# Xjh-UCAS/TAM-TR

Hardware: AMD Instinct MI355X
Metric: images/sec fwd+bwd @640x640 bs=16/GPU (higher is better)
Workload: dtype bf16

## Files before the change

### tam-tr_amd/csrc/bn.hip

```cpp
#include "common.h"

namespace {

constexpr int BN_THREADS = 256;
constexpr int BN_EPT = 16;
constexpr int BN_SLICE = BN_THREADS * BN_EPT;

template <typename T>
__device__ __forceinline__ void ld_slice(const T* __restrict__ p, int n, bool vec, float (&v)[BN_EPT], int (&cnt)) {
  const int base = threadIdx.x * BN_EPT;
  cnt = max(0, min(BN_EPT, n - base));
  if (vec && cnt == BN_EPT) {
#pragma unroll
    for (int q = 0; q < BN_EPT / 4; ++q) {
      float o[4];
      Elt<T>::ld4(p + base + 4 * q, o);
      v[4 * q] = o[0]; v[4 * q + 1] = o[1]; v[4 * q + 2] = o[2]; v[4 * q + 3] = o[3];
    }
  } else {
#pragma unroll
    for (int i = 0; i < BN_EPT; ++i) v[i] = i < cnt ? Elt<T>::ld(p + base + i) : 0.f;
  }
}

// ... 133 lines not shown
    }
  } else {
    for (int i = 0; i < cnt; ++i) Elt<T>::st(y + off + base + i, act_fwd(fmaf(Elt<T>::ld(x + off + base + i) - mean, a, be), act));
  }
}

template <typename T>
__global__ __launch_bounds__(BN_THREADS) void bn_bwd_reduce_kernel(const T* __restrict__ gy, const T* __restrict__ x,
                                                                    const float* __restrict__ mean_rstd, const float* __restrict__ gamma,
                                                                    const float* __restrict__ beta, float* __restrict__ part, int C,
                                                                    int HW, int vec, int act) {
  __shared__ float s_red[BN_THREADS / WAVE];
  const int s = blockIdx.x, c = blockIdx.y, b = blockIdx.z, S = gridDim.x * gridDim.z;
  const int n = min(BN_SLICE, HW - s * BN_SLICE);
  const size_t off = ((size_t)b * C + c) * HW + (size_t)s * BN_SLICE;
  const float mean = mean_rstd[2 * c], rstd = mean_rstd[2 * c + 1], g = gamma[c], be = beta[c];
  float xv[BN_EPT], gv[BN_EPT];
  int cnt;
  ld_slice<T>(x + off, n, vec, xv, cnt);
  ld_slice<T>(gy + off, n, vec, gv, cnt);
  float s1 = 0.f, s2 = 0.f;
#pragma unroll
  for (int i = 0; i < BN_EPT; ++i) {
    if (i < cnt) {
      const float xh = (xv[i] - mean) * rstd;
      const float dz = gv[i] * act_bwd(fmaf(xh, g, be), act);
      s1 += dz;
      s2 = fmaf(dz, xh, s2);
    }
  }
  s1 = block_sum(s1, s_red);
  s2 = block_sum(s2, s_red);
  if (threadIdx.x == 0) {
    float* o = part + ((size_t)c * S + (size_t)b * gridDim.x + s) * 2;
    o[0] = s1; o[1] = s2;
  }
}

template <typename T>
__global__ __launch_bounds__(BN_THREADS) void bn_bwd_apply_kernel(const T* __restrict__ gy, const T* __restrict__ x,
                                                                   const float* __restrict__ mean_rstd, const float* __restrict__ gamma,
                                                                   const float* __restrict__ beta, const float* __restrict__ part,
                                                                   T* __restrict__ gx, float* __restrict__ ggamma, float* __restrict__ gbeta,
                                                                   int C, int HW, int vec, int act, float inv_count) {
  __shared__ float s_red[BN_THREADS / WAVE];
  const int s = blockIdx.x, c = blockIdx.y, b = blockIdx.z, S = gridDim.x * gridDim.z;
  float p1 = 0.f, p2 = 0.f;
  for (int i = threadIdx.x; i < S; i += BN_THREADS) { p1 += part[((size_t)c * S + i) * 2]; p2 += part[((size_t)c * S + i) * 2 + 1]; }
  const float sum_dz = block_sum(p1, s_red), sum_dzx = block_sum(p2, s_red);
  if (s == 0 && b == 0 && threadIdx.x == 0) { ggamma[c] = sum_dzx; gbeta[c] = sum_dz; }
  const int n = min(BN_SLICE, HW - s * BN_SLICE);
  const size_t off = ((size_t)b * C + c) * HW + (size_t)s * BN_SLICE;
  const float mean = mean_rstd[2 * c], rstd = mean_rstd[2 * c + 1], g = gamma[c], be = beta[c];
  const float k1 = sum_dz * inv_count, k2 = sum_dzx * inv_count, gr = g * rstd;
  const int base = threadIdx.x * BN_EPT;
  const int cnt = max(0, min(BN_EPT, n - base));
  if (vec && cnt == BN_EPT) {
#pragma unroll
    for (int q = 0; q < BN_EPT / 4; ++q) {
      float xv[4], gv[4], o[4];
      Elt<T>::ld4(x + off + base + 4 * q, xv);
      Elt<T>::ld4(gy + off + base + 4 * q, gv);
#pragma unroll
      for (int i = 0; i < 4; ++i) {
        const float xh = (xv[i] - mean) * rstd;
        const float dz = gv[i] * act_bwd(fmaf(xh, g, be), act);
        o[i] = gr * (dz - k1 - xh * k2);
      }
      Elt<T>::st4(gx + off + base + 4 * q, o);
    }
  } else {
    for (int i = 0; i < cnt; ++i) {
      const float xh = (Elt<T>::ld(x + off + base + i) - mean) * rstd;
      const float dz = Elt<T>::ld(gy + off + base + i) * act_bwd(fmaf(xh, g, be), act);
      Elt<T>::st(gx + off + base + i, gr * (dz - k1 - xh * k2));
    }
  }
}

template <typename T, int V>
struct Vec;
template <>
struct Vec<float, 4> {
  static __device__ __forceinline__ void ld(const float* p, float (&o)[4]) { Elt<float>::ld4(p, o); }
  static __device__ __forceinline__ void st(float* p, const float (&v)[4]) { Elt<float>::st4(p, v); }
};
template <>
struct Vec<bf16_t, 4> {
  static __device__ __forceinline__ void ld(const bf16_t* p, float (&o)[4]) { Elt<bf16_t>::ld4(p, o); }
  static __device__ __forceinline__ void st(bf16_t* p, const float (&v)[4]) { Elt<bf16_t>::st4(p, v); }
};
template <>
struct Vec<bf16_t, 8> {
  static __device__ __forceinline__ void ld(const bf16_t* p, float (&o)[8]) {
    const uint4 t = *reinterpret_cast<const uint4*>(p);
    const uint32_t w[4] = {t.x, t.y, t.z, t.w};
#pragma unroll
    for (int i = 0; i < 4; ++i) { o[2 * i] = __uint_as_float(w[i] << 16); o[2 * i + 1] = __uint_as_float(w[i] & 0xffff0000u); }
  }
  static __device__ __forceinline__ void st(bf16_t* p, const float (&v)[8]) {
    uint32_t w[4];
#pragma unroll
    for (int i = 0; i < 4; ++i) w[i] = (uint32_t)f2bf(v[2 * i]) | ((uint32_t)f2bf(v[2 * i + 1]) << 16);
    *reinterpret_cast<uint4*>(p) = make_uint4(w[0], w[1], w[2], w[3]);
  }
};

constexpr int CL_UNROLL = 4;

template <int W>
__device__ __forceinline__ void fold_row_lanes(const float (&mine)[W], float* s_acc, float* s_col, int cg) {
#pragma unroll
  for (int j = 0; j < W; ++j) s_acc[threadIdx.x * W + j] = mine[j];
  __syncthreads();
  const int rl = BN_THREADS / cg;
  for (int o = threadIdx.x; o < cg * W; o += BN_THREADS) {
    const int g = o / W, j = o % W;
    float a = 0.f;
    for (int q = 0; q < rl; ++q) a += s_acc[(q * cg + g) * W + j];
    s_col[o] = a;
  }
  __syncthreads();
}

struct Seg { unsigned rows; size_t pitch; };
__device__ __forceinline__ size_t seg_addr(size_t e, int C, int cshift, size_t ld, Seg sg) {
  const size_t row = e >> cshift, col = e & (size_t)(C - 1);
  if (!sg.rows) return row * ld + col;
  const unsigned img = (unsigned)row / sg.rows;
  return (size_t)img * sg.pitch + ((unsigned)row - img * sg.rows) * ld + col;
}

template <typename T, int V>
__global__ __launch_bounds__(BN_THREADS) void bncl_stats_kernel(const T* __restrict__ x, float* __restrict__ part, size_t total, int C,
                                                                 int iters) {
  __shared__ float s_acc[BN_THREADS * 2 * V];
  __shared__ float s_col[2 * 1024];
  const size_t piece = (size_t)BN_THREADS * V, start = (size_t)blockIdx.x * iters * piece, end = min(total, start + iters * piece);
  const int cg = C / V, g = threadIdx.x % cg, S = gridDim.x;
  const T* home = x + start + (size_t)g * V;
  float k[V], acc[2 * V];
  Vec<T, V>::ld(home, k);
#pragma unroll
  for (int j = 0; j < 2 * V; ++j) acc[j] = 0.f;
  const size_t e0 = start + (size_t)threadIdx.x * V;
  for (int it = 0; it < iters; it += CL_UNROLL) {
    float v[CL_UNROLL][V];
#pragma unroll
    for (int u = 0; u < CL_UNROLL; ++u) {
      const size_t e = e0 + (size_t)(it + u) * piece;
      Vec<T, V>::ld(e < end ? x + e : home, v[u]);
    }
#pragma unroll
    for (int u = 0; u < CL_UNROLL; ++u)
#pragma unroll
      for (int j = 0; j < V; ++j) { const float d = v[u][j] - k[j]; acc[j] += d; acc[V + j] = fmaf(d, d, acc[V + j]); }
  }
  fold_row_lanes<2 * V>(acc, s_acc, s_col, cg);
  const float n = (float)((end - start) / C);
  for (int c = threadIdx.x; c < C; c += BN_THREADS) {
    const float s1 = s_col[(c / V) * 2 * V + c % V], s2 = s_col[(c / V) * 2 * V + V + c % V], m = s1 / n;
    float* o = part + ((size_t)c * S + blockIdx.x) * 3;
    o[0] = n; o[1] = Elt<T>::ld(x + start + c) + m; o[2] = s2 - s1 * m;
  }
}

template <typename T, int V>
__global__ __launch_bounds__(BN_THREADS) void bncl_apply_kernel(const T* __restrict__ x, const float* __restrict__ mean_rstd,
                                                                 const float* __restrict__ gamma, const float* __restrict__ beta,
                                                                 const T* __restrict__ res, T* __restrict__ y, size_t total, int C, int iters,
                                                                 int act, Seg ysg = Seg{0, 0}, int cshift = 0) {
  const size_t piece = (size_t)BN_THREADS * V, start = (size_t)blockIdx.x * iters * piece, end = min(total, start + iters * piece);
  const int c0 = (threadIdx.x % (C / V)) * V;
  const size_t home = start + c0;
  float mean[V], a[V], be[V];
#pragma unroll
  for (int j = 0; j < V; ++j) { mean[j] = mean_rstd[2 * (c0 + j)]; a[j] = mean_rstd[2 * (c0 + j) + 1] * gamma[c0 + j]; be[j] = beta[c0 + j]; }
  const size_t e0 = start + (size_t)threadIdx.x * V;
  for (int it = 0; it < iters; it += CL_UNROLL) {
    float v[CL_UNROLL][V];
#pragma unroll
    for (int u = 0; u < CL_UNROLL; ++u) {
      const size_t e = e0 + (size_t)(it + u) * piece;
      Vec<T, V>::ld(x + (e < end ? e : home), v[u]);
    }
#pragma unroll
    for (int u = 0; u < CL_UNROLL; ++u) {
      const size_t e = e0 + (size_t)(it + u) * piece;
#pragma unroll
      for (int j = 0; j < V; ++j) v[u][j] = act_fwd(fmaf(v[u][j] - mean[j], a[j], be[j]), act);
      if (res && e < end) {
        float r[V];
        Vec<T, V>::ld(res + e, r);
#pragma unroll
        for (int j = 0; j < V; ++j) v[u][j] += r[j];
      }
      if (e < end) Vec<T, V>::st(y + (ysg.rows ? seg_addr(e, C, cshift, (size_t)C, ysg) : e), v[u]);
    }
  }
}

template <typename T, int V>
__global__ __launch_bounds__(BN_THREADS) void bncl2_apply_kernel(const T* __restrict__ x1, const T* __restrict__ x2,
                                                                  const float* __restrict__ mr1, const float* __restrict__ mr2,
                                                                  const float* __restrict__ g1, const float* __restrict__ b1,
                                                                  const float* __restrict__ g2, const float* __restrict__ b2,
                                                                  T* __restrict__ y, size_t total, int C, int iters, int act) {
  const size_t piece = (size_t)BN_THREADS * V, start = (size_t)blockIdx.x * iters * piece, end = min(total, start + iters * piece);
  const int c0 = (threadIdx.x % (C / V)) * V;
  const size_t home = start + c0;
  float m1[V], a1[V], m2[V], a2[V], be[V];
#pragma unroll
  for (int j = 0; j < V; ++j) {
    m1[j] = mr1[2 * (c0 + j)]; a1[j] = mr1[2 * (c0 + j) + 1] * g1[c0 + j];
    m2[j] = mr2[2 * (c0 + j)]; a2[j] = mr2[2 * (c0 + j) + 1] * g2[c0 + j];
    be[j] = b1[c0 + j] + b2[c0 + j];
  }
  const size_t e0 = start + (size_t)threadIdx.x * V;
  for (int it = 0; it < iters; it += CL_UNROLL) {
    float v[CL_UNROLL][V], w[CL_UNROLL][V];
#pragma unroll
    for (int u = 0; u < CL_UNROLL; ++u) {
      const size_t e = e0 + (size_t)(it + u) * piece, ee = e < end ? e : home;
      Vec<T, V>::ld(x1 + ee, v[u]);
      Vec<T, V>::ld(x2 + ee, w[u]);
    }
#pragma unroll
    for (int u = 0; u < CL_UNROLL; ++u) {
      const size_t e = e0 + (size_t)(it + u) * piece;
#pragma unroll
      for (int j = 0; j < V; ++j) v[u][j] = act_fwd(fmaf(w[u][j] - m2[j], a2[j], fmaf(v[u][j] - m1[j], a1[j], be[j])), act);
      if (e < end) Vec<T, V>::st(y + e, v[u]);
    }
  }
}

template <typename T, int V>
__global__ __launch_bounds__(BN_THREADS) void bncl2_bwd_reduce_kernel(const T* __restrict__ gy, const T* __restrict__ x1, const T* __restrict__ x2,
                                                                       const float* __restrict__ mr1, const float* __restrict__ mr2,
                                                                       const float* __restrict__ g1, const float* __restrict__ b1,
                                                                       const float* __restrict__ g2, const float* __restrict__ b2,
                                                                       float* __restrict__ part, size_t total, int C, int iters, int act,
                                                                       size_t ldgy, int cshift) {
  __shared__ float s_acc[BN_THREADS * 3 * V];
  __shared__ float s_col[3 * 1024];
  const size_t piece = (size_t)BN_THREADS * V, start = (size_t)blockIdx.x * iters * piece, end = min(total, start + iters * piece);
  const int cg = C / V, c0 = (threadIdx.x % cg) * V, S = gridDim.x;
  const size_t home = start + c0;
  float m1[V], r1[V], m2[V], r2[V], ga1[V], ga2[V], be[V], acc[3 * V];
#pragma unroll
  for (int j = 0; j < V; ++j) {
    m1[j] = mr1[2 * (c0 + j)]; r1[j] = mr1[2 * (c0 + j) + 1]; m2[j] = mr2[2 * (c0 + j)]; r2[j] = mr2[2 * (c0 + j) + 1];
    ga1[j] = g1[c0 + j]; ga2[j] = g2[c0 + j]; be[j] = b1[c0 + j] + b2[c0 + j];
    acc[j] = 0.f; acc[V + j] = 0.f; acc[2 * V + j] = 0.f;
  }
  const size_t e0 = start + (size_t)threadIdx.x * V;
  for (int it = 0; it < iters; it += CL_UNROLL) {
    float xa[CL_UNROLL][V], xb[CL_UNROLL][V], gv[CL_UNROLL][V];
#pragma unroll
    for (int u = 0; u < CL_UNROLL; ++u) {
      const size_t e = e0 + (size_t)(it + u) * piece, ee = e < end ? e : home;
      Vec<T, V>::ld(x1 + ee, xa[u]);
      Vec<T, V>::ld(x2 + ee, xb[u]);
      Vec<T, V>::ld(gy + (ee >> cshift) * ldgy + (ee & (size_t)(C - 1)), gv[u]);
    }
#pragma unroll
    for (int u = 0; u < CL_UNROLL; ++u) {
      const float live = e0 + (size_t)(it + u) * piece < end ? 1.f : 0.f;
#pragma unroll
      for (int j = 0; j < V; ++j) {
        const float h1 = (xa[u][j] - m1[j]) * r1[j], h2 = (xb[u][j] - m2[j]) * r2[j];
        const float dz = live * gv[u][j] * act_bwd(fmaf(h2, ga2[j], fmaf(h1, ga1[j], be[j])), act);
        acc[j] += dz; acc[V + j] = fmaf(dz, h1, acc[V + j]); acc[2 * V + j] = fmaf(dz, h2, acc[2 * V + j]);
      }
    }
  }
  fold_row_lanes<3 * V>(acc, s_acc, s_col, cg);
  for (int c = threadIdx.x; c < C; c += BN_THREADS) {
    float* o = part + ((size_t)c * S + blockIdx.x) * 3;
    o[0] = s_col[(c / V) * 3 * V + c % V]; o[1] = s_col[(c / V) * 3 * V + V + c % V]; o[2] = s_col[(c / V) * 3 * V + 2 * V + c % V];
  }
}

__global__ __launch_bounds__(BN_THREADS) void bncl2_sum_kernel(const float* __restrict__ part, float* __restrict__ sums, float* __restrict__ gg1,
                                                                float* __restrict__ gb1, float* __restrict__ gg2, float* __restrict__ gb2, int S) {
  __shared__ float s_red[BN_THREADS / WAVE];
  const int c = blockIdx.x;
  float a = 0.f, b = 0.f, d = 0.f;
  for (int s = threadIdx.x; s < S; s += BN_THREADS) {
    const float* p = part + ((size_t)c * S + s) * 3;
    a += p[0]; b += p[1]; d += p[2];
  }
  a = block_sum(a, s_red); b = block_sum(b, s_red); d = block_sum(d, s_red);
  if (threadIdx.x == 0) { sums[3 * c] = a; sums[3 * c + 1] = b; sums[3 * c + 2] = d; gb1[c] = a; gb2[c] = a; gg1[c] = b; gg2[c] = d; }
}

template <typename T, int V>
__global__ __launch_bounds__(BN_THREADS) void bncl2_bwd_apply_kernel(const T* __restrict__ gy, const T* __restrict__ x1, const T* __restrict__ x2,
                                                                      const float* __restrict__ mr1, const float* __restrict__ mr2,
                                                                      const float* __restrict__ g1, const float* __restrict__ b1,
                                                                      const float* __restrict__ g2, const float* __restrict__ b2,
                                                                      const float* __restrict__ sums, T* __restrict__ gx1, T* __restrict__ gx2,
                                                                      size_t total, int C, int iters, int act, float inv_count, size_t ldgy,
                                                                      int cshift) {
  const size_t piece = (size_t)BN_THREADS * V, start = (size_t)blockIdx.x * iters * piece, end = min(total, start + iters * piece);
  const int c0 = (threadIdx.x % (C / V)) * V;
  const size_t home = start + c0;
  float m1[V], r1[V], m2[V], r2[V], ga1[V], ga2[V], be[V], k1[V], k2[V], k3[V];
#pragma unroll
  for (int j = 0; j < V; ++j) {
    m1[j] = mr1[2 * (c0 + j)]; r1[j] = mr1[2 * (c0 + j) + 1]; m2[j] = mr2[2 * (c0 + j)]; r2[j] = mr2[2 * (c0 + j) + 1];
    ga1[j] = g1[c0 + j]; ga2[j] = g2[c0 + j]; be[j] = b1[c0 + j] + b2[c0 + j];
    k1[j] = sums[3 * (c0 + j)] * inv_count; k2[j] = sums[3 * (c0 + j) + 1] * inv_count; k3[j] = sums[3 * (c0 + j) + 2] * inv_count;
  }
  const size_t e0 = start + (size_t)threadIdx.x * V;
  for (int it = 0; it < iters; it += CL_UNROLL / 2) {
    float xa[CL_UNROLL / 2][V], xb[CL_UNROLL / 2][V], gv[CL_UNROLL / 2][V];
#pragma unroll
    for (int u = 0; u < CL_UNROLL / 2; ++u) {
      const size_t e = e0 + (size_t)(it + u) * piece, ee = e < end ? e : home;
      Vec<T, V>::ld(x1 + ee, xa[u]);
      Vec<T, V>::ld(x2 + ee, xb[u]);
      Vec<T, V>::ld(gy + (ee >> cshift) * ldgy + (ee & (size_t)(C - 1)), gv[u]);
    }
#pragma unroll
    for (int u = 0; u < CL_UNROLL / 2; ++u) {
      const size_t e = e0 + (size_t)(it + u) * piece;
#pragma unroll
      for (int j = 0; j < V; ++j) {
        const float h1 = (xa[u][j] - m1[j]) * r1[j], h2 = (xb[u][j] - m2[j]) * r2[j];
        const float dz = gv[u][j] * act_bwd(fmaf(h2, ga2[j], fmaf(h1, ga1[j], be[j])), act);
        xa[u][j] = ga1[j] * r1[j] * (dz - k1[j] - h1 * k2[j]);
        xb[u][j] = ga2[j] * r2[j] * (dz - k1[j] - h2 * k3[j]);
      }
      if (e < end) { Vec<T, V>::st(gx1 + e, xa[u]); Vec<T, V>::st(gx2 + e, xb[u]); }
    }
  }
}

template <typename T, int V>
__global__ __launch_bounds__(BN_THREADS) void bncl_bwd_reduce_kernel(const T* __restrict__ gy, const T* __restrict__ x,
                                                                      const float* __restrict__ mean_rstd, const float* __restrict__ gamma,
                                                                      const float* __restrict__ beta, float* __restrict__ part, size_t total,
                                                                      int C, int iters, int act, size_t ldgy, int cshift, Seg gsg = Seg{0, 0}) {
  __shared__ float s_acc[BN_THREADS * 2 * V];
  __shared__ float s_col[2 * 1024];
  const size_t piece = (size_t)BN_THREADS * V, start = (size_t)blockIdx.x * iters * piece, end = min(total, start + iters * piece);
  const int cg = C / V, c0 = (threadIdx.x % cg) * V, S = gridDim.x;
  const size_t home = start + c0;
  float mean[V], rstd[V], gm[V], be[V], acc[2 * V];
#pragma unroll
  for (int j = 0; j < V; ++j) {
    mean[j] = mean_rstd[2 * (c0 + j)]; rstd[j] = mean_rstd[2 * (c0 + j) + 1]; gm[j] = gamma[c0 + j]; be[j] = beta[c0 + j];
    acc[j] = 0.f; acc[V + j] = 0.f;
  }
  const size_t e0 = start + (size_t)threadIdx.x * V;
  for (int it = 0; it < iters; it += CL_UNROLL) {
    float xv[CL_UNROLL][V], gv[CL_UNROLL][V];
#pragma unroll
    for (int u = 0; u < CL_UNROLL; ++u) {
      const size_t e = e0 + (size_t)(it + u) * piece, ee = e < end ? e : home;
      Vec<T, V>::ld(x + ee, xv[u]);
      Vec<T, V>::ld(gy + seg_addr(ee, C, cshift, ldgy, gsg), gv[u]);
    }
#pragma unroll
    for (int u = 0; u < CL_UNROLL; ++u) {
      const float live = e0 + (size_t)(it + u) * piece < end ? 1.f : 0.f;
#pragma unroll
      for (int j = 0; j < V; ++j) {
        const float xh = (xv[u][j] - mean[j]) * rstd[j];
        const float dz = live * gv[u][j] * act_bwd(fmaf(xh, gm[j], be[j]), act);
        acc[j] += dz; acc[V + j] = fmaf(dz, xh, acc[V + j]);
      }
    }
  }
  fold_row_lanes<2 * V>(acc, s_acc, s_col, cg);
  for (int c = threadIdx.x; c < C; c += BN_THREADS) {
    float* o = part + ((size_t)c * S + blockIdx.x) * 2;
    o[0] = s_col[(c / V) * 2 * V + c % V]; o[1] = s_col[(c / V) * 2 * V + V + c % V];
  }
}

__global__ __launch_bounds__(BN_THREADS) void bncl_sum_kernel(const float* __restrict__ part, float* __restrict__ sums, float* __restrict__ ggamma,
                                                               float* __restrict__ gbeta, int S) {
  __shared__ float s_red[BN_THREADS / WAVE];
  const int c = blockIdx.x;
  float a = 0.f, b = 0.f;
  for (int s = threadIdx.x; s < S; s += BN_THREADS) { a += part[((size_t)c * S + s) * 2]; b += part[((size_t)c * S + s) * 2 + 1]; }
  a = block_sum(a, s_red); b = block_sum(b, s_red);
  if (threadIdx.x == 0) { sums[2 * c] = a; sums[2 * c + 1] = b; gbeta[c] = a; ggamma[c] = b; }
}

template <typename T, int V>
__global__ __launch_bounds__(BN_THREADS) void bncl_bwd_apply_kernel(const T* __restrict__ gy, const T* __restrict__ x,
                                                                     const float* __restrict__ mean_rstd, const float* __restrict__ gamma,
                                                                     const float* __restrict__ beta, const float* __restrict__ sums,
                                                                     T* __restrict__ gx, size_t total, int C, int iters, int act,
                                                                     float inv_count, size_t ldgy, int cshift, Seg gsg = Seg{0, 0}) {
  const size_t piece = (size_t)BN_THREADS * V, start = (size_t)blockIdx.x * iters * piece, end = min(total, start + iters * piece);
  const int c0 = (threadIdx.x % (C / V)) * V;
  const size_t home = start + c0;
  float mean[V], rstd[V], gm[V], be[V], k1[V], k2[V];
#pragma unroll
  for (int j = 0; j < V; ++j) {
    mean[j] = mean_rstd[2 * (c0 + j)]; rstd[j] = mean_rstd[2 * (c0 + j) + 1]; gm[j] = gamma[c0 + j]; be[j] = beta[c0 + j];
    k1[j] = sums[2 * (c0 + j)] * inv_count; k2[j] = sums[2 * (c0 + j) + 1] * inv_count;
  }
  const size_t e0 = start + (size_t)threadIdx.x * V;
  for (int it = 0; it < iters; it += CL_UNROLL) {
    float xv[CL_UNROLL][V], gv[CL_UNROLL][V];
#pragma unroll
    for (int u = 0; u < CL_UNROLL; ++u) {
      const size_t e = e0 + (size_t)(it + u) * piece, ee = e < end ? e : home;
      Vec<T, V>::ld(x + ee, xv[u]);
      Vec<T, V>::ld(gy + seg_addr(ee, C, cshift, ldgy, gsg), gv[u]);
    }
#pragma unroll
    for (int u = 0; u < CL_UNROLL; ++u) {
      const size_t e = e0 + (size_t)(it + u) * piece;
#pragma unroll
      for (int j = 0; j < V; ++j) {
        const float xh = (xv[u][j] - mean[j]) * rstd[j];
        const float dz = gv[u][j] * act_bwd(fmaf(xh, gm[j], be[j]), act);
        gv[u][j] = gm[j] * rstd[j] * (dz - k1[j] - xh * k2[j]);
      }
      if (e < end) Vec<T, V>::st(gx + e, gv[u]);
    }
  }
}

}

extern "C" int tamtr_bn_slices(int B, int HW) { return B * ((HW + BN_SLICE - 1) / BN_SLICE); }

static int bn_check(const void* a, const void* b, int B, int C, int HW, int dtype, int act) {
  if (!a || !b || B <= 0 || C <= 0 || HW <= 0) return TAMTR_EINVAL;
  if ((dtype != TAMTR_F32 && dtype != TAMTR_BF16) || (act != 0 && act != 1)) return TAMTR_EINVAL;
  if (B > 65535 || C > 65535) return TAMTR_EUNSUP;
  return TAMTR_OK;
}
static int bn_vec(const void* p, const void* q, int HW, int dtype) {
  const int e = dtype == TAMTR_F32 ? 4 : 2;
  return HW % 4 == 0 && ((uintptr_t)p % (4 * e)) == 0 && (!q || ((uintptr_t)q % (4 * e)) == 0);
}

extern "C" int tamtr_bn_act_fwd(const void* x, const float* gamma, const float* beta, float* running_mean, float* running_var, void* y,
                                float* mean_rstd, float* partials, int B, int C, int HW, float eps, float momentum, int act, int dtype,
                                void* stream) {
  const int rc = bn_check(x, y, B, C, HW, dtype, act);
  if (rc) return rc;
  if (!gamma || !beta || !mean_rstd || !partials) return TAMTR_EINVAL;
  const int sh = (HW + BN_SLICE - 1) / BN_SLICE, vec = bn_vec(x, y, HW, dtype);
  const dim3 grid(sh, C, B);
  hipStream_t s = (hipStream_t)stream;
  if (dtype == TAMTR_F32) hipLaunchKernelGGL(bn_stats_kernel<float>, grid, dim3(BN_THREADS), 0, s, (const float*)x, partials, C, HW, vec);
  else hipLaunchKernelGGL(bn_stats_kernel<bf16_t>, grid, dim3(BN_THREADS), 0, s, (const bf16_t*)x, partials, C, HW, vec);
  if (dtype == TAMTR_F32)
    hipLaunchKernelGGL(bn_apply_kernel<float>, grid, dim3(BN_THREADS), 0, s, (const float*)x, partials, mean_rstd, running_mean, running_var,
                       gamma, beta, (float*)y, C, HW, vec, act, eps, momentum);
  else
    hipLaunchKernelGGL(bn_apply_kernel<bf16_t>, grid, dim3(BN_THREADS), 0, s, (const bf16_t*)x, partials, mean_rstd, running_mean,
                       running_var, gamma, beta, (bf16_t*)y, C, HW, vec, act, eps, momentum);
  return tamtr_launch_status();
}

extern "C" int tamtr_bn_act_bwd(const void* gy, const void* x, const float* gamma, const float* beta, const float* mean_rstd, void* gx,
                                float* ggamma, float* gbeta, float* partials, int B, int C, int HW, int act, int dtype, void* stream) {
  const int rc = bn_check(gy, x, B, C, HW, dtype, act);
  if (rc) return rc;
  if (!gamma || !beta || !mean_rstd || !gx || !ggamma || !gbeta || !partials) return TAMTR_EINVAL;
  const int sh = (HW + BN_SLICE - 1) / BN_SLICE, vec = bn_vec(x, gy, HW, dtype) && bn_vec(gx, nullptr, HW, dtype);
  const dim3 grid(sh, C, B);
  hipStream_t s = (hipStream_t)stream;
  const float inv = 1.f / ((float)B * (float)HW);
  if (dtype == TAMTR_F32) {
    hipLaunchKernelGGL(bn_bwd_reduce_kernel<float>, grid, dim3(BN_THREADS), 0, s, (const float*)gy, (const float*)x, mean_rstd, gamma, beta,
                       partials, C, HW, vec, act);
    hipLaunchKernelGGL(bn_bwd_apply_kernel<float>, grid, dim3(BN_THREADS), 0, s, (const float*)gy, (const float*)x, mean_rstd, gamma, beta,
                       partials, (float*)gx, ggamma, gbeta, C, HW, vec, act, inv);
  } else {
    hipLaunchKernelGGL(bn_bwd_reduce_kernel<bf16_t>, grid, dim3(BN_THREADS), 0, s, (const bf16_t*)gy, (const bf16_t*)x, mean_rstd, gamma,
                       beta, partials, C, HW, vec, act);
    hipLaunchKernelGGL(bn_bwd_apply_kernel<bf16_t>, grid, dim3(BN_THREADS), 0, s, (const bf16_t*)gy, (const bf16_t*)x, mean_rstd, gamma,
                       beta, partials, (bf16_t*)gx, ggamma, gbeta, C, HW, vec, act, inv);
  }
  return tamtr_launch_status();
}

static int bncl_vec(int C, int dtype) { return dtype == TAMTR_BF16 && C % 8 == 0 ? 8 : 4; }
static int bncl_iters(long long N, int C, int dtype) {
  const long long piece = (long long)BN_THREADS * bncl_vec(C, dtype), total = N * C;
  const long long it = (total / piece / 1024 + CL_UNROLL - 1) / CL_UNROLL * CL_UNROLL;
  return (int)(it < 4 ? 4 : it > 64 ? 64 : it);
}
extern "C" int tamtr_bncl_blocks(long long N, int C, int dtype) {
  if (N <= 0 || C <= 0) return 0;
  const long long chunk = (long long)bncl_iters(N, C, dtype) * BN_THREADS * bncl_vec(C, dtype);
  return (int)((N * C + chunk - 1) / chunk);
}

static int bncl_check(const void* a, const void* b, long long N, int C, int dtype, int act) {
  if (!a || !b || N <= 0 || C <= 0) return TAMTR_EINVAL;
  if ((dtype != TAMTR_F32 && dtype != TAMTR_BF16) || (act != 0 && act != 1)) return TAMTR_EINVAL;
  const int cg = C / bncl_vec(C, dtype);
  if (C % 4 || C > 1024 || cg > BN_THREADS || (BN_THREADS % cg) || N > 2000000000LL / C) return TAMTR_EUNSUP;
  if (((uintptr_t)a | (uintptr_t)b) % 16) return TAMTR_EUNSUP;
  return TAMTR_OK;
}

static int bncl_act_fwd_impl(const void* x, const float* gamma, const float* beta, float* running_mean, float* running_var,
                             const void* residual, void* y, float* mean_rstd, float* partials, long long N, int C, float eps,
                             float momentum, int act, int dtype, void* stream, Seg ysg, int cshift) {
  const int rc = bncl_check(x, y, N, C, dtype, act);
  if (rc) return rc;
  if (!gamma || !beta || !mean_rstd || !partials) return TAMTR_EINVAL;
  if (residual && (uintptr_t)residual % 16) return TAMTR_EUNSUP;
  const int S = tamtr_bncl_blocks(N, C, dtype), V = bncl_vec(C, dtype), iters = bncl_iters(N, C, dtype);
  const size_t total = (size_t)N * C;
  hipStream_t s = (hipStream_t)stream;
  if (dtype == TAMTR_F32) hipLaunchKernelGGL((bncl_stats_kernel<float, 4>), dim3(S), dim3(BN_THREADS), 0, s, (const float*)x, partials, total, C, iters);
  else if (V == 8) hipLaunchKernelGGL((bncl_stats_kernel<bf16_t, 8>), dim3(S), dim3(BN_THREADS), 0, s, (const bf16_t*)x, partials, total, C, iters);
  else hipLaunchKernelGGL((bncl_stats_kernel<bf16_t, 4>), dim3(S), dim3(BN_THREADS), 0, s, (const bf16_t*)x, partials, total, C, iters);
  hipLaunchKernelGGL(bn_finalize_kernel, dim3(C), dim3(BN_THREADS), 0, s, partials, mean_rstd, running_mean, running_var, S, eps, momentum);
  if (dtype == TAMTR_F32)
    hipLaunchKernelGGL((bncl_apply_kernel<float, 4>), dim3(S), dim3(BN_THREADS), 0, s, (const float*)x, mean_rstd, gamma, beta, (const float*)residual, (float*)y, total, C, iters, act, ysg, cshift);
  else if (V == 8)
    hipLaunchKernelGGL((bncl_apply_kernel<bf16_t, 8>), dim3(S), dim3(BN_THREADS), 0, s, (const bf16_t*)x, mean_rstd, gamma, beta, (const bf16_t*)residual, (bf16_t*)y, total, C, iters, act, ysg, cshift);
  else
    hipLaunchKernelGGL((bncl_apply_kernel<bf16_t, 4>), dim3(S), dim3(BN_THREADS), 0, s, (const bf16_t*)x, mean_rstd, gamma, beta, (const bf16_t*)residual, (bf16_t*)y, total, C, iters, act, ysg, cshift);
  return tamtr_launch_status();
}

extern "C" int tamtr_bncl_act_fwd(const void* x, const float* gamma, const float* beta, float* running_mean, float* running_var,
                                  const void* residual, void* y, float* mean_rstd, float* partials, long long N, int C, float eps,
                                  float momentum, int act, int dtype, void* stream) {
  return bncl_act_fwd_impl(x, gamma, beta, running_mean, running_var, residual, y, mean_rstd, partials, N, C, eps, momentum, act, dtype, stream,
                           Seg{0, 0}, 0);
}

extern "C" int tamtr_bncl_act_seg_fwd(const void* x, const float* gamma, const float* beta, float* running_mean, float* running_var, void* y,
                                      long long seg_rows, long long seg_pitch, float* mean_rstd, float* partials, long long N, int C, float eps,
                                      float momentum, int act, int dtype, void* stream) {
  if (seg_rows <= 0 || N % seg_rows || seg_pitch < seg_rows * C || seg_pitch % 8 || (C & (C - 1)) || seg_rows > 0x7fffffffLL) return TAMTR_EUNSUP;
  int cshift = 0;
  while ((1 << cshift) < C) ++cshift;
  return bncl_act_fwd_impl(x, gamma, beta, running_mean, running_var, nullptr, y, mean_rstd, partials, N, C, eps, momentum, act, dtype, stream,
                           Seg{(unsigned)seg_rows, (size_t)seg_pitch}, cshift);
}

static int bncl_act_bwd_impl(const void* gy, long long ldgy, const void* x, const float* gamma, const float* beta,
                             const float* mean_rstd, void* gx, float* ggamma, float* gbeta, float* partials, long long N, int C, int act,
                             int dtype, void* stream, Seg gsg) {
  const int rc = bncl_check(gy, x, N, C, dtype, act);
  if (rc) return rc;
  if (ldgy < C || ldgy % bncl_vec(C, dtype) || (C & (C - 1))) return TAMTR_EUNSUP;
  int cshift = 0;
  while ((1 << cshift) < C) ++cshift;
  if (!gamma || !beta || !mean_rstd || !gx || !ggamma || !gbeta || !partials || (uintptr_t)gx % 16) return TAMTR_EINVAL;
  const int S = tamtr_bncl_blocks(N, C, dtype), V = bncl_vec(C, dtype), iters = bncl_iters(N, C, dtype);
  const size_t total = (size_t)N * C;
  hipStream_t s = (hipStream_t)stream;
  float* sums = partials + (size_t)C * S * 2;
  const float inv = 1.f / (float)N;
  if (dtype == TAMTR_F32)
    hipLaunchKernelGGL((bncl_bwd_reduce_kernel<float, 4>), dim3(S), dim3(BN_THREADS), 0, s, (const float*)gy, (const float*)x, mean_rstd, gamma, beta, partials, total, C, iters, act, (size_t)ldgy, cshift, gsg);
  else if (V == 8)
    hipLaunchKernelGGL((bncl_bwd_reduce_kernel<bf16_t, 8>), dim3(S), dim3(BN_THREADS), 0, s, (const bf16_t*)gy, (const bf16_t*)x, mean_rstd, gamma, beta, partials, total, C, iters, act, (size_t)ldgy, cshift, gsg);
  else
    hipLaunchKernelGGL((bncl_bwd_reduce_kernel<bf16_t, 4>), dim3(S), dim3(BN_THREADS), 0, s, (const bf16_t*)gy, (const bf16_t*)x, mean_rstd, gamma, beta, partials, total, C, iters, act, (size_t)ldgy, cshift, gsg);
  hipLaunchKernelGGL(bncl_sum_kernel, dim3(C), dim3(BN_THREADS), 0, s, partials, sums, ggamma, gbeta, S);
  if (dtype == TAMTR_F32)
    hipLaunchKernelGGL((bncl_bwd_apply_kernel<float, 4>), dim3(S), dim3(BN_THREADS), 0, s, (const float*)gy, (const float*)x, mean_rstd, gamma, beta, sums, (float*)gx, total, C, iters, act, inv, (size_t)ldgy, cshift, gsg);
  else if (V == 8)
    hipLaunchKernelGGL((bncl_bwd_apply_kernel<bf16_t, 8>), dim3(S), dim3(BN_THREADS), 0, s, (const bf16_t*)gy, (const bf16_t*)x, mean_rstd, gamma, beta, sums, (bf16_t*)gx, total, C, iters, act, inv, (size_t)ldgy, cshift, gsg);
  else
    hipLaunchKernelGGL((bncl_bwd_apply_kernel<bf16_t, 4>), dim3(S), dim3(BN_THREADS), 0, s, (const bf16_t*)gy, (const bf16_t*)x, mean_rstd, gamma, beta, sums, (bf16_t*)gx, total, C, iters, act, inv, (size_t)ldgy, cshift, gsg);
  return tamtr_launch_status();
}

extern "C" int tamtr_bncl_act_bwd(const void* gy, long long ldgy, const void* x, const float* gamma, const float* beta,
                                  const float* mean_rstd, void* gx, float* ggamma, float* gbeta, float* partials, long long N, int C, int act,
                                  int dtype, void* stream) {
  return bncl_act_bwd_impl(gy, ldgy, x, gamma, beta, mean_rstd, gx, ggamma, gbeta, partials, N, C, act, dtype, stream, Seg{0, 0});
}

extern "C" int tamtr_bncl_act_seg_bwd(const void* gy, long long seg_rows, long long seg_pitch, const void* x, const float* gamma, const float* beta,
                                      const float* mean_rstd, void* gx, float* ggamma, float* gbeta, float* partials, long long N, int C, int act,
                                      int dtype, void* stream) {
  if (seg_rows <= 0 || N % seg_rows || seg_pitch < seg_rows * C || seg_pitch % 8 || seg_rows > 0x7fffffffLL) return TAMTR_EUNSUP;
  return bncl_act_bwd_impl(gy, C, x, gamma, beta, mean_rstd, gx, ggamma, gbeta, partials, N, C, act, dtype, stream,
                           Seg{(unsigned)seg_rows, (size_t)seg_pitch});
}

extern "C" int tamtr_bncl2_act_fwd(const void* x1, const float* gamma1, const float* beta1, float* running_mean1, float* running_var1,
                                   const void* x2, const float* gamma2, const float* beta2, float* running_mean2, float* running_var2,
                                   void* y, float* mean_rstd, float* partials, long long N, int C, float eps, float momentum, int act,
                                   int dtype, void* stream) {
  int rc = bncl_check(x1, y, N, C, dtype, act);
  if (!rc) rc = bncl_check(x2, y, N, C, dtype, act);
  if (rc) return rc;
  if (!gamma1 || !beta1 || !gamma2 || !beta2 || !mean_rstd || !partials) return TAMTR_EINVAL;
  const int S = tamtr_bncl_blocks(N, C, dtype), V = bncl_vec(C, dtype), iters = bncl_iters(N, C, dtype);
  const size_t total = (size_t)N * C;
  hipStream_t s = (hipStream_t)stream;
  float* mr2 = mean_rstd + 2 * (size_t)C;
  float* part2 = partials + (size_t)C * S * 3;
#define STATS(T, VV, X, P) hipLaunchKernelGGL((bncl_stats_kernel<T, VV>), dim3(S), dim3(BN_THREADS), 0, s, (const T*)X, P, total, C, iters)
#define APPLY(T, VV)                                                                                                                   \
  hipLaunchKernelGGL((bncl2_apply_kernel<T, VV>), dim3(S), dim3(BN_THREADS), 0, s, (const T*)x1, (const T*)x2, mean_rstd, mr2, gamma1, beta1, \
                     gamma2, beta2, (T*)y, total, C, iters, act)
  if (dtype == TAMTR_F32) { STATS(float, 4, x1, partials); STATS(float, 4, x2, part2); }
  else if (V == 8) { STATS(bf16_t, 8, x1, partials); STATS(bf16_t, 8, x2, part2); }
  else { STATS(bf16_t, 4, x1, partials); STATS(bf16_t, 4, x2, part2); }
  hipLaunchKernelGGL(bn_finalize_kernel, dim3(C), dim3(BN_THREADS), 0, s, partials, mean_rstd, running_mean1, running_var1, S, eps, momentum);
  hipLaunchKernelGGL(bn_finalize_kernel, dim3(C), dim3(BN_THREADS), 0, s, part2, mr2, running_mean2, running_var2, S, eps, momentum);
  if (dtype == TAMTR_F32) APPLY(float, 4); else if (V == 8) APPLY(bf16_t, 8); else APPLY(bf16_t, 4);
#undef STATS
#undef APPLY
  return tamtr_launch_status();
}

extern "C" int tamtr_bncl2_act_bwd(const void* gy, long long ldgy, const void* x1, const void* x2, const float* gamma1, const float* beta1,
                                   const float* gamma2, const float* beta2, const float* mean_rstd, void* gx1, void* gx2, float* ggamma1,
                                   float* gbeta1, float* ggamma2, float* gbeta2, float* partials, long long N, int C, int act, int dtype,
                                   void* stream) {
  int rc = bncl_check(gy, x1, N, C, dtype, act);
  if (!rc) rc = bncl_check(x2, gx1, N, C, dtype, act);
  if (rc) return rc;
  if (!gamma1 || !beta1 || !gamma2 || !beta2 || !mean_rstd || !gx2 || !ggamma1 || !gbeta1 || !ggamma2 || !gbeta2 || !partials ||
      (uintptr_t)gx2 % 16)
    return TAMTR_EINVAL;
  if (ldgy < C || ldgy % bncl_vec(C, dtype) || (C & (C - 1))) return TAMTR_EUNSUP;
  int cshift = 0;
  while ((1 << cshift) < C) ++cshift;
  const int S = tamtr_bncl_blocks(N, C, dtype), V = bncl_vec(C, dtype), iters = bncl_iters(N, C, dtype);
  const size_t total = (size_t)N * C;
  hipStream_t s = (hipStream_t)stream;
  const float* mr2 = mean_rstd + 2 * (size_t)C;
  float* sums = partials + (size_t)C * S * 3;
  const float inv = 1.f / (float)N;
#define RED(T, VV)                                                                                                                       \
  hipLaunchKernelGGL((bncl2_bwd_reduce_kernel<T, VV>), dim3(S), dim3(BN_THREADS), 0, s, (const T*)gy, (const T*)x1, (const T*)x2, mean_rstd, mr2, \
                     gamma1, beta1, gamma2, beta2, partials, total, C, iters, act, (size_t)ldgy, cshift)
#define APP(T, VV)                                                                                                                       \
  hipLaunchKernelGGL((bncl2_bwd_apply_kernel<T, VV>), dim3(S), dim3(BN_THREADS), 0, s, (const T*)gy, (const T*)x1, (const T*)x2, mean_rstd, mr2,  \
                     gamma1, beta1, gamma2, beta2, sums, (T*)gx1, (T*)gx2, total, C, iters, act, inv, (size_t)ldgy, cshift)
  if (dtype == TAMTR_F32) RED(float, 4); else if (V == 8) RED(bf16_t, 8); else RED(bf16_t, 4);
  hipLaunchKernelGGL(bncl2_sum_kernel, dim3(C), dim3(BN_THREADS), 0, s, partials, sums, ggamma1, gbeta1, ggamma2, gbeta2, S);
  if (dtype == TAMTR_F32) APP(float, 4); else if (V == 8) APP(bf16_t, 8); else APP(bf16_t, 4);
#undef RED
#undef APP
  return tamtr_launch_status();
}

// ... 23 lines not shown
```

Before: 213.8.

## Software-pipeline channels-last BN reduce loads with register ring and XCD chunk remap

Replaces the load-all-then-reduce unrolled loops in the channels-last BN stats and backward-reduce kernels with a register ring of raw vector loads. Loads for later pieces are issued while earlier ones are converted and reduced, so memory latency overlaps with arithmetic. It also remaps block index to chunk so that consecutive chunks land on the same XCD (blockIdx % 8). It adds waves-per-EU occupancy hints and keeps the stats kernel's shift values in shared memory instead of reloading them from global. Many compile-time ablation switches are added; they are off by default, and the change risks higher register pressure.

Measured after the change: 214.9 (median of 6 runs). No clear change (+0.5%).

```diff
diff --git a/tam-tr_amd/csrc/bn.hip b/tam-tr_amd/csrc/bn.hip
--- a/tam-tr_amd/csrc/bn.hip
+++ b/tam-tr_amd/csrc/bn.hip
@@ -239,22 +239,33 @@
 struct Vec;
 template <>
 struct Vec<float, 4> {
-  static __device__ __forceinline__ void ld(const float* p, float (&o)[4]) { Elt<float>::ld4(p, o); }
+  using Raw = float4;
+  static __device__ __forceinline__ Raw ldr(const float* p) { return *reinterpret_cast<const float4*>(p); }
+  static __device__ __forceinline__ void cvt(const Raw& t, float (&o)[4]) { o[0] = t.x; o[1] = t.y; o[2] = t.z; o[3] = t.w; }
+  static __device__ __forceinline__ void ld(const float* p, float (&o)[4]) { cvt(ldr(p), o); }
   static __device__ __forceinline__ void st(float* p, const float (&v)[4]) { Elt<float>::st4(p, v); }
 };
 template <>
 struct Vec<bf16_t, 4> {
-  static __device__ __forceinline__ void ld(const bf16_t* p, float (&o)[4]) { Elt<bf16_t>::ld4(p, o); }
+  using Raw = uint2;
+  static __device__ __forceinline__ Raw ldr(const bf16_t* p) { return *reinterpret_cast<const uint2*>(p); }
+  static __device__ __forceinline__ void cvt(const Raw& t, float (&o)[4]) {
+    o[0] = __uint_as_float(t.x << 16); o[1] = __uint_as_float(t.x & 0xffff0000u);
+    o[2] = __uint_as_float(t.y << 16); o[3] = __uint_as_float(t.y & 0xffff0000u);
+  }
+  static __device__ __forceinline__ void ld(const bf16_t* p, float (&o)[4]) { cvt(ldr(p), o); }
   static __device__ __forceinline__ void st(bf16_t* p, const float (&v)[4]) { Elt<bf16_t>::st4(p, v); }
 };
 template <>
 struct Vec<bf16_t, 8> {
-  static __device__ __forceinline__ void ld(const bf16_t* p, float (&o)[8]) {
-    const uint4 t = *reinterpret_cast<const uint4*>(p);
+  using Raw = uint4;
+  static __device__ __forceinline__ Raw ldr(const bf16_t* p) { return *reinterpret_cast<const uint4*>(p); }
+  static __device__ __forceinline__ void cvt(const Raw& t, float (&o)[8]) {
     const uint32_t w[4] = {t.x, t.y, t.z, t.w};
 #pragma unroll
     for (int i = 0; i < 4; ++i) { o[2 * i] = __uint_as_float(w[i] << 16); o[2 * i + 1] = __uint_as_float(w[i] & 0xffff0000u); }
   }
+  static __device__ __forceinline__ void ld(const bf16_t* p, float (&o)[8]) { cvt(ldr(p), o); }
   static __device__ __forceinline__ void st(bf16_t* p, const float (&v)[8]) {
     uint32_t w[4];
 #pragma unroll
@@ -274,10 +285,81 @@
   for (int o = threadIdx.x; o < cg * W; o += BN_THREADS) {
     const int g = o / W, j = o % W;
     float a = 0.f;
+#pragma unroll 8
     for (int q = 0; q < rl; ++q) a += s_acc[(q * cg + g) * W + j];
     s_col[o] = a;
   }
   __syncthreads();
+}
+
+#ifndef BNCL_DEPTH
+#define BNCL_DEPTH 4
+#endif
+#ifndef BNCL_RING_BYTES
+#define BNCL_RING_BYTES 64
+#endif
+#ifndef BNCL_WAVES
+#define BNCL_WAVES 4
+#endif
+constexpr int CL_DEPTH = BNCL_DEPTH, CL_RING_BYTES = BNCL_RING_BYTES;
+constexpr int cl_depth(int streams, int raw_bytes) {
+  int d = 2;
+  while (2 * d <= CL_DEPTH && streams * 2 * d * raw_bytes <= CL_RING_BYTES) d *= 2;
+  return d;
+}
+#define CL_WAVES(n) __attribute__((amdgpu_waves_per_eu((n) < BNCL_WAVES ? (n) : BNCL_WAVES)))
+template <int D, typename Issue, typename Reduce>
+__device__ __forceinline__ void cl_stream(int iters, Issue issue, Reduce reduce) {
+  static_assert(D % CL_UNROLL == 0 || CL_UNROLL % D == 0, "the ring divides a round of CL_UNROLL pieces or holds whole rounds");
+#ifdef BNCL_ABL_SERIAL
+  constexpr int R = D < CL_UNROLL ? D : CL_UNROLL;
+  for (int it = 0; it < iters; it += R) {
+#pragma unroll
+    for (int u = 0; u < R; ++u) issue(u, it + u);
+#pragma unroll
+    for (int u = 0; u < R; ++u) reduce(u, it + u);
+  }
+#else
+#pragma unroll
+  for (int u = 0; u < D; ++u) issue(u, u);
+  int it = 0;
+  for (; it + D < iters; it += D) {
+#pragma unroll
+    for (int u = 0; u < D; ++u) { reduce(u, it + u); issue(u, it + D + u); }
+  }
+#pragma unroll
+  for (int u = 0; u < D; ++u)
+    if (CL_UNROLL % D == 0 || it + u < iters) reduce(u, it + u);
+#endif
+}
+template <typename T, int V>
+__device__ __forceinline__ typename Vec<T, V>::Raw cl_ldr(const T* p) {
+#ifdef BNCL_ABL_NOLOAD
+  typename Vec<T, V>::Raw r;
+  __builtin_memset(&r, (int)((uintptr_t)p >> 4 & 63), sizeof(r));
+  return r;
+#else
+  return Vec<T, V>::ldr(p);
+#endif
+}
+__device__ __forceinline__ float cl_act_bwd(float z, int act) {
+#ifdef BNCL_ABL_NOACT
+  return 1.f + 0.f * z;
+#else
+  return act_bwd(z, act);
+#endif
+}
+template <int W>
+__device__ __forceinline__ bool cl_abl_nofold(const float (&acc)[W], float* part) {
+#ifdef BNCL_ABL_NOFOLD
+  float t = 0.f;
+#pragma unroll
+  for (int j = 0; j < W; ++j) t += acc[j];
+  if (t == 12345.678f) part[0] = t;
+  return true;
+#else
+  return false;
+#endif
 }
 
 struct Seg { unsigned rows; size_t pitch; };
@@ -288,12 +370,23 @@
   return (size_t)img * sg.pitch + ((unsigned)row - img * sg.rows) * ld + col;
 }
 
+__device__ __forceinline__ int cl_chunk() {
+#ifdef BNCL_ABL_NOREMAP
+  return blockIdx.x;
+#else
+  const int S = gridDim.x, lab = blockIdx.x % 8, q = S / 8, r = S % 8;
+  return (lab < r ? lab * (q + 1) : r * (q + 1) + (lab - r) * q) + blockIdx.x / 8;
+#endif
+}
+
 template <typename T, int V>
-__global__ __launch_bounds__(BN_THREADS) void bncl_stats_kernel(const T* __restrict__ x, float* __restrict__ part, size_t total, int C,
+__global__ __launch_bounds__(BN_THREADS) CL_WAVES(4) void bncl_stats_kernel(const T* __restrict__ x, float* __restrict__ part, size_t total, int C,
                                                                  int iters) {
   __shared__ float s_acc[BN_THREADS * 2 * V];
   __shared__ float s_col[2 * 1024];
-  const size_t piece = (size_t)BN_THREADS * V, start = (size_t)blockIdx.x * iters * piece, end = min(total, start + iters * piece);
+  __shared__ float s_k[1024];
+  const int chunk = cl_chunk();
+  const size_t piece = (size_t)BN_THREADS * V, start = (size_t)chunk * iters * piece, end = min(total, start + iters * piece);
   const int cg = C / V, g = threadIdx.x % cg, S = gridDim.x;
   const T* home = x + start + (size_t)g * V;
   float k[V], acc[2 * V];
@@ -301,24 +394,34 @@
 #pragma unroll
   for (int j = 0; j < 2 * V; ++j) acc[j] = 0.f;
   const size_t e0 = start + (size_t)threadIdx.x * V;
-  for (int it = 0; it < iters; it += CL_UNROLL) {
-    float v[CL_UNROLL][V];
-#pragma unroll
-    for (int u = 0; u < CL_UNROLL; ++u) {
-      const size_t e = e0 + (size_t)(it + u) * piece;
-      Vec<T, V>::ld(e < end ? x + e : home, v[u]);
-    }
-#pragma unroll
-    for (int u = 0; u < CL_UNROLL; ++u)
-#pragma unroll
-      for (int j = 0; j < V; ++j) { const float d = v[u][j] - k[j]; acc[j] += d; acc[V + j] = fmaf(d, d, acc[V + j]); }
+  constexpr int D = cl_depth(1, sizeof(typename Vec<T, V>::Raw));
+  typename Vec<T, V>::Raw ring[D];
+  cl_stream<D>(
+      iters,
+      [&](int u, int it) {
+        const size_t e = e0 + (size_t)it * piece;
+        ring[u] = cl_ldr<T, V>(e < end ? x + e : home);
+      },
+      [&](int u, int) {
+        float v[V];
+        Vec<T, V>::cvt(ring[u], v);
+#pragma unroll
+        for (int j = 0; j < V; ++j) { const float d = v[j] - k[j]; acc[j] += d; acc[V + j] = fmaf(d, d, acc[V + j]); }
+      });
+  if (cl_abl_nofold(acc, part)) return;
+  if (threadIdx.x < cg) {
+#pragma unroll
+    for (int j = 0; j < V; ++j) s_k[threadIdx.x * V + j] = k[j];
   }
   fold_row_lanes<2 * V>(acc, s_acc, s_col, cg);
   const float n = (float)((end - start) / C);
   for (int c = threadIdx.x; c < C; c += BN_THREADS) {
     const float s1 = s_col[(c / V) * 2 * V + c % V], s2 = s_col[(c / V) * 2 * V + V + c % V], m = s1 / n;
-    float* o = part + ((size_t)c * S + blockIdx.x) * 3;
-    o[0] = n; o[1] = Elt<T>::ld(x + start + c) + m; o[2] = s2 - s1 * m;
+    float* o = part + ((size_t)c * S + chunk) * 3;
+#ifdef BNCL_ABL_NOSTORE
+    if (m == 12345.678f)
+#endif
+    { o[0] = n; o[1] = s_k[c] + m; o[2] = fmaf(-s1, m, s2); }
   }
 }
 
@@ -327,7 +430,8 @@
                                                                  const float* __restrict__ gamma, const float* __restrict__ beta,
                                                                  const T* __restrict__ res, T* __restrict__ y, size_t total, int C, int iters,
                                                                  int act, Seg ysg = Seg{0, 0}, int cshift = 0) {
-  const size_t piece = (size_t)BN_THREADS * V, start = (size_t)blockIdx.x * iters * piece, end = min(total, start + iters * piece);
+  const int chunk = cl_chunk();
+  const size_t piece = (size_t)BN_THREADS * V, start = (size_t)chunk * iters * piece, end = min(total, start + iters * piece);
   const int c0 = (threadIdx.x % (C / V)) * V;
   const size_t home = start + c0;
   float mean[V], a[V], be[V];
@@ -363,7 +467,8 @@
                                                                   const float* __restrict__ g1, const float* __restrict__ b1,
                                                                   const float* __restrict__ g2, const float* __restrict__ b2,
                                                                   T* __restrict__ y, size_t total, int C, int iters, int act) {
-  const size_t piece = (size_t)BN_THREADS * V, start = (size_t)blockIdx.x * iters * piece, end = min(total, start + iters * piece);
+  const int chunk = cl_chunk();
+  const size_t piece = (size_t)BN_THREADS * V, start = (size_t)chunk * iters * piece, end = min(total, start + iters * piece);
   const int c0 = (threadIdx.x % (C / V)) * V;
   const size_t home = start + c0;
   float m1[V], a1[V], m2[V], a2[V], be[V];
@@ -393,7 +498,7 @@
 }
 
 template <typename T, int V>
-__global__ __launch_bounds__(BN_THREADS) void bncl2_bwd_reduce_kernel(const T* __restrict__ gy, const T* __restrict__ x1, const T* __restrict__ x2,
+__global__ __launch_bounds__(BN_THREADS) CL_WAVES(V == 8 ? 2 : 4) void bncl2_bwd_reduce_kernel(const T* __restrict__ gy, const T* __restrict__ x1, const T* __restrict__ x2,
                                                                        const float* __restrict__ mr1, const float* __restrict__ mr2,
                                                                        const float* __restrict__ g1, const float* __restrict__ b1,
                                                                        const float* __restrict__ g2, const float* __restrict__ b2,
@@ -401,7 +506,8 @@
                                                                        size_t ldgy, int cshift) {
   __shared__ float s_acc[BN_THREADS * 3 * V];
   __shared__ float s_col[3 * 1024];
-  const size_t piece = (size_t)BN_THREADS * V, start = (size_t)blockIdx.x * iters * piece, end = min(total, start + iters * piece);
+  const int chunk = cl_chunk();
+  const size_t piece = (size_t)BN_THREADS * V, start = (size_t)chunk * iters * piece, end = min(total, start + iters * piece);
   const int cg = C / V, c0 = (threadIdx.x % cg) * V, S = gridDim.x;
   const size_t home = start + c0;
   float m1[V], r1[V], m2[V], r2[V], ga1[V], ga2[V], be[V], acc[3 * V];
@@ -412,29 +518,33 @@
     acc[j] = 0.f; acc[V + j] = 0.f; acc[2 * V + j] = 0.f;
   }
   const size_t e0 = start + (size_t)threadIdx.x * V;
-  for (int it = 0; it < iters; it += CL_UNROLL) {
-    float xa[CL_UNROLL][V], xb[CL_UNROLL][V], gv[CL_UNROLL][V];
-#pragma unroll
-    for (int u = 0; u < CL_UNROLL; ++u) {
-      const size_t e = e0 + (size_t)(it + u) * piece, ee = e < end ? e : home;
-      Vec<T, V>::ld(x1 + ee, xa[u]);
-      Vec<T, V>::ld(x2 + ee, xb[u]);
-      Vec<T, V>::ld(gy + (ee >> cshift) * ldgy + (ee & (size_t)(C - 1)), gv[u]);
-    }
-#pragma unroll
-    for (int u = 0; u < CL_UNROLL; ++u) {
-      const float live = e0 + (size_t)(it + u) * piece < end ? 1.f : 0.f;
-#pragma unroll
-      for (int j = 0; j < V; ++j) {
-        const float h1 = (xa[u][j] - m1[j]) * r1[j], h2 = (xb[u][j] - m2[j]) * r2[j];
-        const float dz = live * gv[u][j] * act_bwd(fmaf(h2, ga2[j], fmaf(h1, ga1[j], be[j])), act);
-        acc[j] += dz; acc[V + j] = fmaf(dz, h1, acc[V + j]); acc[2 * V + j] = fmaf(dz, h2, acc[2 * V + j]);
-      }
-    }
-  }
+  constexpr int D = cl_depth(3, sizeof(typename Vec<T, V>::Raw));
+  typename Vec<T, V>::Raw ra[D], rb[D], rg[D];
+  cl_stream<D>(
+      iters,
+      [&](int u, int it) {
+        const size_t e = e0 + (size_t)it * piece, ee = e < end ? e : home;
+        ra[u] = cl_ldr<T, V>(x1 + ee);
+        rb[u] = cl_ldr<T, V>(x2 + ee);
+        rg[u] = cl_ldr<T, V>(gy + (ee >> cshift) * ldgy + (ee & (size_t)(C - 1)));
+      },
+      [&](int u, int it) {
+        float xa[V], xb[V], gv[V];
+        Vec<T, V>::cvt(ra[u], xa);
+        Vec<T, V>::cvt(rb[u], xb);
+        Vec<T, V>::cvt(rg[u], gv);
+        const float live = e0 + (size_t)it * piece < end ? 1.f : 0.f;
+#pragma unroll
+        for (int j = 0; j < V; ++j) {
+          const float h1 = (xa[j] - m1[j]) * r1[j], h2 = (xb[j] - m2[j]) * r2[j];
+          const float dz = live * gv[j] * cl_act_bwd(fmaf(h2, ga2[j], fmaf(h1, ga1[j], be[j])), act);
+          acc[j] += dz; acc[V + j] = fmaf(dz, h1, acc[V + j]); acc[2 * V + j] = fmaf(dz, h2, acc[2 * V + j]);
+        }
+      });
+  if (cl_abl_nofold(acc, part)) return;
   fold_row_lanes<3 * V>(acc, s_acc, s_col, cg);
   for (int c = threadIdx.x; c < C; c += BN_THREADS) {
-    float* o = part + ((size_t)c * S + blockIdx.x) * 3;
+    float* o = part + ((size_t)c * S + chunk) * 3;
     o[0] = s_col[(c / V) * 3 * V + c % V]; o[1] = s_col[(c / V) * 3 * V + V + c % V]; o[2] = s_col[(c / V) * 3 * V + 2 * V + c % V];
   }
 }
@@ -460,7 +570,8 @@
                                                                       const float* __restrict__ sums, T* __restrict__ gx1, T* __restrict__ gx2,
                                                                       size_t total, int C, int iters, int act, float inv_count, size_t ldgy,
                                                                       int cshift) {
-  const size_t piece = (size_t)BN_THREADS * V, start = (size_t)blockIdx.x * iters * piece, end = min(total, start + iters * piece);
+  const int chunk = cl_chunk();
+  const size_t piece = (size_t)BN_THREADS * V, start = (size_t)chunk * iters * piece, end = min(total, start + iters * piece);
   const int c0 = (threadIdx.x % (C / V)) * V;
   const size_t home = start + c0;
   float m1[V], r1[V], m2[V], r2[V], ga1[V], ga2[V], be[V], k1[V], k2[V], k3[V];
@@ -496,13 +607,14 @@
 }
 
 template <typename T, int V>
-__global__ __launch_bounds__(BN_THREADS) void bncl_bwd_reduce_kernel(const T* __restrict__ gy, const T* __restrict__ x,
+__global__ __launch_bounds__(BN_THREADS) CL_WAVES(4) void bncl_bwd_reduce_kernel(const T* __restrict__ gy, const T* __restrict__ x,
                                                                       const float* __restrict__ mean_rstd, const float* __restrict__ gamma,
                                                                       const float* __restrict__ beta, float* __restrict__ part, size_t total,
                                                                       int C, int iters, int act, size_t ldgy, int cshift, Seg gsg = Seg{0, 0}) {
   __shared__ float s_acc[BN_THREADS * 2 * V];
   __shared__ float s_col[2 * 1024];
-  const size_t piece = (size_t)BN_THREADS * V, start = (size_t)blockIdx.x * iters * piece, end = min(total, start + iters * piece);
+  const int chunk = cl_chunk();
+  const size_t piece = (size_t)BN_THREADS * V, start = (size_t)chunk * iters * piece, end = min(total, start + iters * piece);
   const int cg = C / V, c0 = (threadIdx.x % cg) * V, S = gridDim.x;
   const size_t home = start + c0;
   float mean[V], rstd[V], gm[V], be[V], acc[2 * V];
@@ -512,29 +624,35 @@
     acc[j] = 0.f; acc[V + j] = 0.f;
   }
   const size_t e0 = start + (size_t)threadIdx.x * V;
-  for (int it = 0; it < iters; it += CL_UNROLL) {
-    float xv[CL_UNROLL][V], gv[CL_UNROLL][V];
-#pragma unroll
-    for (int u = 0; u < CL_UNROLL; ++u) {
-      const size_t e = e0 + (size_t)(it + u) * piece, ee = e < end ? e : home;
-      Vec<T, V>::ld(x + ee, xv[u]);
-      Vec<T, V>::ld(gy + seg_addr(ee, C, cshift, ldgy, gsg), gv[u]);
-    }
-#pragma unroll
-    for (int u = 0; u < CL_UNROLL; ++u) {
-      const float live = e0 + (size_t)(it + u) * piece < end ? 1.f : 0.f;
-#pragma unroll
-      for (int j = 0; j < V; ++j) {
-        const float xh = (xv[u][j] - mean[j]) * rstd[j];
-        const float dz = live * gv[u][j] * act_bwd(fmaf(xh, gm[j], be[j]), act);
-        acc[j] += dz; acc[V + j] = fmaf(dz, xh, acc[V + j]);
-      }
-    }
-  }
+  constexpr int D = cl_depth(2, sizeof(typename Vec<T, V>::Raw));
+  typename Vec<T, V>::Raw rx[D], rg[D];
+  cl_stream<D>(
+      iters,
+      [&](int u, int it) {
+        const size_t e = e0 + (size_t)it * piece, ee = e < end ? e : home;
+        rx[u] = cl_ldr<T, V>(x + ee);
+        rg[u] = cl_ldr<T, V>(gy + seg_addr(ee, C, cshift, ldgy, gsg));
+      },
+      [&](int u, int it) {
+        float xv[V], gv[V];
+        Vec<T, V>::cvt(rx[u], xv);
+        Vec<T, V>::cvt(rg[u], gv);
+        const float live = e0 + (size_t)it * piece < end ? 1.f : 0.f;
+#pragma unroll
+        for (int j = 0; j < V; ++j) {
+          const float xh = (xv[j] - mean[j]) * rstd[j];
+          const float dz = live * gv[j] * cl_act_bwd(fmaf(xh, gm[j], be[j]), act);
+          acc[j] += dz; acc[V + j] = fmaf(dz, xh, acc[V + j]);
+        }
+      });
+  if (cl_abl_nofold(acc, part)) return;
   fold_row_lanes<2 * V>(acc, s_acc, s_col, cg);
   for (int c = threadIdx.x; c < C; c += BN_THREADS) {
-    float* o = part + ((size_t)c * S + blockIdx.x) * 2;
-    o[0] = s_col[(c / V) * 2 * V + c % V]; o[1] = s_col[(c / V) * 2 * V + V + c % V];
+    float* o = part + ((size_t)c * S + chunk) * 2;
+#ifdef BNCL_ABL_NOSTORE
+    if (s_col[c] == 12345.678f)
+#endif
+    { o[0] = s_col[(c / V) * 2 * V + c % V]; o[1] = s_col[(c / V) * 2 * V + V + c % V]; }
   }
 }
 
@@ -554,7 +672,8 @@
                                                                      const float* __restrict__ beta, const float* __restrict__ sums,
                                                                      T* __restrict__ gx, size_t total, int C, int iters, int act,
                                                                      float inv_count, size_t ldgy, int cshift, Seg gsg = Seg{0, 0}) {
-  const size_t piece = (size_t)BN_THREADS * V, start = (size_t)blockIdx.x * iters * piece, end = min(total, start + iters * piece);
+  const int chunk = cl_chunk();
+  const size_t piece = (size_t)BN_THREADS * V, start = (size_t)chunk * iters * piece, end = min(total, start + iters * piece);
   const int c0 = (threadIdx.x % (C / V)) * V;
   const size_t home = start + c0;
   float mean[V], rstd[V], gm[V], be[V], k1[V], k2[V];
@@ -644,6 +763,10 @@
   return tamtr_launch_status();
 }
 
+#ifndef BNCL_ABL_ONLY
+#define BNCL_ABL_ONLY 0
+#endif
+constexpr bool CL_RUN_REDUCE = BNCL_ABL_ONLY != 2, CL_RUN_APPLY = BNCL_ABL_ONLY != 1;
 static int bncl_vec(int C, int dtype) { return dtype == TAMTR_BF16 && C % 8 == 0 ? 8 : 4; }
 static int bncl_iters(long long N, int C, int dtype) {
   const long long piece = (long long)BN_THREADS * bncl_vec(C, dtype), total = N * C;
@@ -675,11 +798,13 @@
   const int S = tamtr_bncl_blocks(N, C, dtype), V = bncl_vec(C, dtype), iters = bncl_iters(N, C, dtype);
   const size_t total = (size_t)N * C;
   hipStream_t s = (hipStream_t)stream;
-  if (dtype == TAMTR_F32) hipLaunchKernelGGL((bncl_stats_kernel<float, 4>), dim3(S), dim3(BN_THREADS), 0, s, (const float*)x, partials, total, C, iters);
+  if (!CL_RUN_REDUCE) {}
+  else if (dtype == TAMTR_F32) hipLaunchKernelGGL((bncl_stats_kernel<float, 4>), dim3(S), dim3(BN_THREADS), 0, s, (const float*)x, partials, total, C, iters);
   else if (V == 8) hipLaunchKernelGGL((bncl_stats_kernel<bf16_t, 8>), dim3(S), dim3(BN_THREADS), 0, s, (const bf16_t*)x, partials, total, C, iters);
   else hipLaunchKernelGGL((bncl_stats_kernel<bf16_t, 4>), dim3(S), dim3(BN_THREADS), 0, s, (const bf16_t*)x, partials, total, C, iters);
   hipLaunchKernelGGL(bn_finalize_kernel, dim3(C), dim3(BN_THREADS), 0, s, partials, mean_rstd, running_mean, running_var, S, eps, momentum);
-  if (dtype == TAMTR_F32)
+  if (!CL_RUN_APPLY) {}
+  else if (dtype == TAMTR_F32)
     hipLaunchKernelGGL((bncl_apply_kernel<float, 4>), dim3(S), dim3(BN_THREADS), 0, s, (const float*)x, mean_rstd, gamma, beta, (const float*)residual, (float*)y, total, C, iters, act, ysg, cshift);
   else if (V == 8)
     hipLaunchKernelGGL((bncl_apply_kernel<bf16_t, 8>), dim3(S), dim3(BN_THREADS), 0, s, (const bf16_t*)x, mean_rstd, gamma, beta, (const bf16_t*)residual, (bf16_t*)y, total, C, iters, act, ysg, cshift);
@@ -719,14 +844,16 @@
   hipStream_t s = (hipStream_t)stream;
   float* sums = partials + (size_t)C * S * 2;
   const float inv = 1.f / (float)N;
-  if (dtype == TAMTR_F32)
+  if (!CL_RUN_REDUCE) {}
+  else if (dtype == TAMTR_F32)
     hipLaunchKernelGGL((bncl_bwd_reduce_kernel<float, 4>), dim3(S), dim3(BN_THREADS), 0, s, (const float*)gy, (const float*)x, mean_rstd, gamma, beta, partials, total, C, iters, act, (size_t)ldgy, cshift, gsg);
   else if (V == 8)
     hipLaunchKernelGGL((bncl_bwd_reduce_kernel<bf16_t, 8>), dim3(S), dim3(BN_THREADS), 0, s, (const bf16_t*)gy, (const bf16_t*)x, mean_rstd, gamma, beta, partials, total, C, iters, act, (size_t)ldgy, cshift, gsg);
   else
     hipLaunchKernelGGL((bncl_bwd_reduce_kernel<bf16_t, 4>), dim3(S), dim3(BN_THREADS), 0, s, (const bf16_t*)gy, (const bf16_t*)x, mean_rstd, gamma, beta, partials, total, C, iters, act, (size_t)ldgy, cshift, gsg);
   hipLaunchKernelGGL(bncl_sum_kernel, dim3(C), dim3(BN_THREADS), 0, s, partials, sums, ggamma, gbeta, S);
-  if (dtype == TAMTR_F32)
+  if (!CL_RUN_APPLY) {}
+  else if (dtype == TAMTR_F32)
     hipLaunchKernelGGL((bncl_bwd_apply_kernel<float, 4>), dim3(S), dim3(BN_THREADS), 0, s, (const float*)gy, (const float*)x, mean_rstd, gamma, beta, sums, (float*)gx, total, C, iters, act, inv, (size_t)ldgy, cshift, gsg);
   else if (V == 8)
     hipLaunchKernelGGL((bncl_bwd_apply_kernel<bf16_t, 8>), dim3(S), dim3(BN_THREADS), 0, s, (const bf16_t*)gy, (const bf16_t*)x, mean_rstd, gamma, beta, sums, (bf16_t*)gx, total, C, iters, act, inv, (size_t)ldgy, cshift, gsg);
```
